# federicomegler/sq-learn

Hardware: AMD Instinct MI355X
Metric: q-means fit samples/sec (Lloyd samples*iterations/s, delta-means + tomography noise) (higher is better)
Workload: dtype fp32; 1 GPU; model=q-means k=1024 delta=0.5 (10000000 x 256 synthetic), global_batch=10000000, seq_len=256, parallelism=dp1

## Files before the change

sq_learn_amd/csrc/estep_f32.hip:

```cpp
#include "common.h"
#include "band.h"
#include "f16_tile.h"
#include "sq_api.h"

namespace sq {

constexpr int kMaxCand = 16;

#ifndef SQ_SPLIT_ACC_ALL
#define SQ_SPLIT_ACC_ALL 1
#endif
template <int KSD, int TOP = 2>
__global__ void __launch_bounds__(256, 1) estep_f32_kernel(
    const float* __restrict__ X, const _Float16* __restrict__ C, const float* __restrict__ xn,
    int* __restrict__ labels, float* __restrict__ mind, long long* __restrict__ ovf_rows,
    int* __restrict__ ovf_count, double* __restrict__ part, long long n, int k_pad, float alpha,
    float inv_alpha2, float delta_s, RngKey key, long long row_offset, int ovf_cap,
    const long long* __restrict__ rlist, const int* __restrict__ rcount,
    const float* __restrict__ cmax2_p, long long* __restrict__ mrows, int* __restrict__ mcand,
    int* __restrict__ multi_count, unsigned char* __restrict__ xflag, long long mcap) {
  const float Cm = cmax2_p ? sqrtf(*cmax2_p) * (1.0f + 0x1p-16f) : 0.0f;
  constexpr bool SPLIT_ACC = SQ_SPLIT_ACC_ALL || TOP == 3;
  constexpr float kEps3 =
      SPLIT_ACC ? (3.0f * 0x1p-22f + (KSD * 16 + 18.0f) * 0x1p-24f + 2.0f * KSD * 16 * 0x1p-34f) *
// ... 1310 lines not shown
      const unsigned long long pm = __ballot(cin && rank == r) & gmask;
      if (wide && pm) plane = __ffsll((long long)pm) - 1;
      dmin_w = mine ? dme : __builtin_inff();
#pragma unroll
      for (int o = 1; o < LPR; o <<= 1) dmin_w = fminf(dmin_w, __shfl_xor(dmin_w, o, 64));
    }
    const int pick = __shfl(cur.myj, plane, 64);
    const float hpick = __shfl(hi, plane, 64);
    const float dpick = __shfl(dme, plane, 64);
    float lo_o = (mine && lane != plane) ? lo : __builtin_inff();
#pragma unroll
    for (int o = 1; o < LPR; o <<= 1) lo_o = fminf(lo_o, __shfl_xor(lo_o, o, 64));
    fix(nxt);
    ldrow(Cm + (size_t)nxt.j0 * DX, c0n);
    ldrow(Cm + (size_t)nxt.j1 * DX, c1n);
    __builtin_amdgcn_sched_barrier(0);
    labels[g] = pick;
    if constexpr (UB) ub[g] = sqrtf(hpick) * (1.0f + 0x1p-20f);
    if (wide && sub == 0 && corr) corr[g] = dmin_w - dpick;
    xflag[e] = done_any ? 0 : 1;
    if (rec) {
      const float dpl = __shfl(dme, plane, 64), spl = __shfl(slack, plane, 64);
      const float gc = mine ? dme - dpl : 0.0f;
      float ge = mine ? slack + spl + fabsf(gc) * 0x1p-23f : 0.0f;
#pragma unroll
      for (int o = 1; o < LPR; o <<= 1) ge = fmaxf(ge, __shfl_xor(ge, o, 64));
      const int w = sub & 7;
      const float gw = __shfl(gc, gbase + min(max(w - 2, 0), LPR - 1), 64);
      const float v = w == 0 ? dpl : (w == 1 ? ge : gw);
      const unsigned i0 = (unsigned)__shfl(cur.myj, gbase, 64) & 0x3FFFu;
      const unsigned i1 = (unsigned)__shfl(cur.myj, gbase + 1, 64) & 0x3FFFu;
      const unsigned i2 = (unsigned)__shfl(cur.myj, gbase + 2, 64) & 0x3FFFu;
      const unsigned i3 = (unsigned)__shfl(cur.myj, gbase + 3, 64) & 0x3FFFu;
      const unsigned cm1 = (unsigned)min(max(c_r, 1), kGapCand) - 1u;
      const unsigned id0 = i0 | ((unsigned)(plane - gbase) & 3u) << 14 |
                           (c_r > 1 ? i1 : i0) << 16 | cm1 << 30;
      const unsigned id1 = (c_r > 2 ? i2 : i0) | (c_r > 3 ? i3 : i0) << 16;
      float* rw = reinterpret_cast<float*>(rec + g) + w;
      if (w < 6) *rw = v;
      else *reinterpret_cast<unsigned*>(rw) = w == 6 ? id0 : id1;
      if (sub == 0) rec_it[g] = (done && c_r <= kGapCand) ? it_now + 2 : 1;
    }
    __builtin_amdgcn_sched_barrier(0);
    g2 = g3;
    g3 = g4;
  };
  for (long long st = 0; st < nsteps; st += 2) {
    step(st, rA, xA, c0A, c1A, rB, xB, c0B, c1B);
    if (st + 1 >= nsteps) break;
    step(st + 1, rB, xB, c0B, c1B, rA, xA, c0A, c1A);
  }
}

typedef _Float16 gs_h2 __attribute__((ext_vector_type(2)));
__device__ __forceinline__ float gs_dot(const uint4 a, const uint4 b, float acc) {
  acc = __builtin_amdgcn_fdot2(__builtin_bit_cast(gs_h2, a.x), __builtin_bit_cast(gs_h2, b.x), acc,
                               false);
  acc = __builtin_amdgcn_fdot2(__builtin_bit_cast(gs_h2, a.y), __builtin_bit_cast(gs_h2, b.y), acc,
                               false);
  acc = __builtin_amdgcn_fdot2(__builtin_bit_cast(gs_h2, a.z), __builtin_bit_cast(gs_h2, b.z), acc,
                               false);
  acc = __builtin_amdgcn_fdot2(__builtin_bit_cast(gs_h2, a.w), __builtin_bit_cast(gs_h2, b.w), acc,
                               false);
  return acc;
}
__device__ __forceinline__ float gs_dot(const uint2 a, const uint2 b, float acc) {
  acc = __builtin_amdgcn_fdot2(__builtin_bit_cast(gs_h2, a.x), __builtin_bit_cast(gs_h2, b.x), acc,
                               false);
  acc = __builtin_amdgcn_fdot2(__builtin_bit_cast(gs_h2, a.y), __builtin_bit_cast(gs_h2, b.y), acc,
                               false);
  return acc;
}
__device__ __forceinline__ uint4 gs_zero(uint4) { return make_uint4(0u, 0u, 0u, 0u); }
template <int CTRL>
__device__ __forceinline__ float gs_dpp_add(float v) {
  return v + __int_as_float(__builtin_amdgcn_update_dpp(0, __float_as_int(v), CTRL, 0xF, 0xF,
                                                         false));
}
__device__ __forceinline__ uint2 gs_zero(uint2) { return make_uint2(0u, 0u); }

template <int DX>
__global__ void __launch_bounds__(256) gap_screen_kernel(
    const _Float16* __restrict__ Xh, const float* __restrict__ xn,
    const long long* __restrict__ mrows_b, const int* __restrict__ count_b,
    const _Float16* __restrict__ dsh, long long dsh_stride, const float* __restrict__ dq,
    long long dq_stride, float inv_alpha, float delta, int* __restrict__ labels,
    GapRec* __restrict__ rec, int* __restrict__ mflag, int it_now, int ring, int rebase_age,
    long long* __restrict__ mrows, int* __restrict__ multi_count, long long cap,
    int* __restrict__ n_done, long long* __restrict__ mrows_mv, int* __restrict__ count_mv) {
  constexpr int LPR = 32;
  using VT = typename std::conditional<DX % 256 == 0, uint4, uint2>::type;
  constexpr int HV = (int)sizeof(VT) / 2;
  constexpr int V = DX / (LPR * HV);
  static_assert(DX % 128 == 0 && V >= 1, "gap screen: d_pad multiple of 128");
  const int lane = threadIdx.x & 63;
  const int sub = lane & (LPR - 1);
  const bool hi = lane >= LPR;
  const long long cnt = min((long long)*count_b, cap);
  const long long gw = (long long)blockIdx.x * (blockDim.x >> 6) + (threadIdx.x >> 6);
  const long long nw = (long long)gridDim.x * (blockDim.x >> 6);
  const long long nblk = (cnt + 63) / 64;
  const float sub_err = sqrtf((float)DX) * 0x1p-25f * inv_alpha;
  constexpr float gam = (float)(DX + 16) * 0x1p-24f;
  uint32_t done_cnt = 0;
  constexpr int kGapStage = 256;
  __shared__ long long stage_fw[4][kGapStage], stage_mv[4][kGapStage];
  int n_fw = 0, n_mv = 0;
  auto flush = [&](const long long* buf, int& cnt, long long* __restrict__ dst, int* counter) {
    if (cnt == 0) return;
    int b = 0;
    if (lane == 0) b = atomicAdd(counter, cnt);
    b = __shfl(b, 0, 64);
    __builtin_amdgcn_wave_barrier();
    for (int i = lane; i < cnt; i += 64)
      if ((long long)b + i < cap) dst[(long long)b + i] = buf[i];
    cnt = 0;
  };
  auto stage = [&](bool pred, long long row, long long* buf, int& cnt, long long* __restrict__ dst,
                   int* counter) {
    const unsigned long long pm = __ballot(pred);
    if (pm == 0) return;
    if (cnt + 64 > kGapStage) flush(buf, cnt, dst, counter);
    if (pred) buf[cnt + __popcll(pm & ((1ull << lane) - 1ull))] = row;
    cnt += __popcll(pm);
  };
  auto rl = [](int v, int l) -> int { return __builtin_amdgcn_readlane(v, l); };
  auto rlf = [](float v, int l) -> float {
    return __int_as_float(__builtin_amdgcn_readlane(__float_as_int(v), l));
  };
  for (long long blk = gw; blk < nblk; blk += nw) {
    const long long e = blk * 64 + lane;
    const bool live = e < cnt;
    const long long g = mrows_b[live ? e : cnt - 1];
    const int base_it = mflag[g] - 2;
    const int rslot = base_it % ring, age = it_now - base_it;
    const float4* rp = reinterpret_cast<const float4*>(rec + g);
    const float4 r0 = rp[0], r1 = rp[1];
    const float xq = xn[g];
    const unsigned id0 = __float_as_uint(r1.z), id1 = __float_as_uint(r1.w);
    const int c_r = (int)(id0 >> 30) + 1, slot = (int)((id0 >> 14) & 3u);
    int jc[kGapCand];
    jc[0] = (int)(id0 & 0x3FFFu);
    jc[1] = (int)((id0 >> 16) & 0x3FFFu);
    jc[2] = (int)(id1 & 0x3FFFu);
    jc[3] = (int)((id1 >> 16) & 0x3FFFu);
    const float* dqs = dq + (size_t)rslot * dq_stride;
    float4 d0[kGapCand];
    float inv[kGapCand];
#pragma unroll
    for (int c = 0; c < kGapCand; ++c) {
      d0[c] = reinterpret_cast<const float4*>(dqs)[2 * jc[c]];
      inv[c] = dqs[8 * jc[c] + 4];
    }
    float y[kGapCand] = {0.0f, 0.0f, 0.0f, 0.0f};
    constexpr int NB = 4;
    VT xv[NB][V], sv[NB][kGapCand][V];
    int pcm[NB];
    auto issue = [&](int p, int b) {
      const int ra = 2 * p, rb = 2 * p + 1;
      const long long ga = ((long long)rl((int)(g >> 32), ra) << 32) | (unsigned)rl((int)g, ra);
      const long long gb = ((long long)rl((int)(g >> 32), rb) << 32) | (unsigned)rl((int)g, rb);
      const long long gm = hi ? gb : ga;
      const VT* xr = reinterpret_cast<const VT*>(Xh + (size_t)gm * DX);
#pragma unroll
      for (int q = 0; q < V; ++q) xv[b][q] = xr[q * LPR + sub];
      const int sa = rl(rslot, ra), sb = rl(rslot, rb);
      const _Float16* ds = dsh + (size_t)(hi ? sb : sa) * dsh_stride;
      pcm[b] = max(rl(c_r, ra), rl(c_r, rb));
#pragma unroll
      for (int c = 0; c < kGapCand; ++c) {
        if (c < 2 || c < pcm[b]) {
          const int j = hi ? rl(jc[c], rb) : rl(jc[c], ra);
          const VT* sr = reinterpret_cast<const VT*>(ds + (size_t)j * DX);
#pragma unroll
          for (int q = 0; q < V; ++q) sv[b][c][q] = sr[q * LPR + sub];
        } else {
#pragma unroll
          for (int q = 0; q < V; ++q) sv[b][c][q] = gs_zero(VT{});
        }
      }
    };
    auto consume = [&](int p, int b) {
#pragma unroll
      for (int c = 0; c < kGapCand; ++c) {
        if (c < 2 || c < pcm[b]) {
          float acc = 0.0f;
#pragma unroll
          for (int q = 0; q < V; ++q) acc = gs_dot(xv[b][q], sv[b][c][q], acc);
          acc = gs_dpp_add<0xB1>(acc);
          acc = gs_dpp_add<0x4E>(acc);
          acc = gs_dpp_add<0x141>(acc);
          acc = gs_dpp_add<0x140>(acc);
          const float a = rlf(acc, 0) + rlf(acc, 16), bb = rlf(acc, 32) + rlf(acc, 48);
          y[c] = lane == 2 * p ? a : (lane == 2 * p + 1 ? bb : y[c]);
        }
      }
    };
#pragma unroll
    for (int b = 0; b < NB - 1; ++b) issue(b, b);
#pragma unroll 1
    for (int p = 0; p < 32; p += NB) {
#pragma unroll
      for (int b = 0; b < NB; ++b) {
        if (p + b + NB - 1 < 32) issue(p + b + NB - 1, (b + NB - 1) % NB);
        consume(p + b, b);
      }
    }
    const float nx = sqrtf(xq) * (1.0f + 0x1p-16f);
    const float ex = 0x1p-11f * nx + sub_err, nxh = nx + ex;
    float yr[kGapCand], E[kGapCand], qv[kGapCand];
#pragma unroll
    for (int c = 0; c < kGapCand; ++c) {
      yr[c] = y[c] * inv[c];
      E[c] = ex * d0[c].z + nxh * (d0[c].w + gam * (d0[c].z + d0[c].w)) + d0[c].y;
      qv[c] = d0[c].x;
    }
    float ya = 0.0f, Ea = 0.0f, qa = 0.0f;
#pragma unroll
    for (int c = 0; c < kGapCand; ++c)
      if (c == slot) {
        ya = yr[c];
        Ea = E[c];
        qa = qv[c];
      }
    const float gold[kGapCand] = {r0.z, r0.w, r1.x, r1.y};
    float gn[kGapCand], gmax = 0.0f, Emax = 0.0f, ymax = fabsf(ya), qmax = fabsf(qa);
#pragma unroll
    for (int c = 0; c < kGapCand; ++c) {
      const bool in = c < c_r;
      gn[c] = in ? (c == slot ? 0.0f : gold[c] + 2.0f * (ya - yr[c]) + (qv[c] - qa))
                 : __builtin_inff();
      if (in) {
        gmax = fmaxf(gmax, fabsf(gold[c]));
        Emax = fmaxf(Emax, E[c]);
        ymax = fmaxf(ymax, fabsf(yr[c]));
        qmax = fmaxf(qmax, fabsf(qv[c]));
      }
    }
    const float da = r0.x - 2.0f * ya + qa;
    float err = r0.y + 2.0f * (Ea + Emax) +
                0x1p-22f * (fmaxf(gmax, fabsf(r0.x)) + 4.0f * ymax + 2.0f * qmax);
    err *= 1.0f + 0x1p-20f;
    int m = 0;
    float gm = gn[0];
#pragma unroll
    for (int c = 1; c < kGapCand; ++c)
      if (gn[c] < gm) {
        gm = gn[c];
        m = c;
      }
    bool done = live && c_r >= 2 && slot < c_r && err < 0.25f * delta + 1.0f;
    float gmx = 0.0f;
#pragma unroll
    for (int c = 0; c < kGapCand; ++c)
      if (c < c_r && c != m) {
        done = done && (gn[c] - gm > delta + 2.0f * err);
        gmx = fmaxf(gmx, gn[c]);
      }
    if (done && (m != slot || age >= rebase_age)) {
      const float da_n = da + gm;
      float err_n =
          (m == slot ? err : 2.0f * err) + 0x1p-22f * (gmx + fabsf(da_n) + fabsf(gm));
      err_n *= 1.0f + 0x1p-20f;
      float gr[kGapCand];
#pragma unroll
      for (int c = 0; c < kGapCand; ++c) gr[c] = c < c_r ? gn[c] - gm : 0.0f;
      float4* wp = reinterpret_cast<float4*>(rec + g);
      wp[0] = make_float4(da_n, err_n, gr[0], gr[1]);
      wp[1] = make_float4(gr[2], gr[3],
                          __uint_as_float((id0 & ~(3u << 14)) | (unsigned)m << 14),
                          __uint_as_float(id1));
      if (m != slot) labels[g] = jc[0] * (m == 0) + jc[1] * (m == 1) + jc[2] * (m == 2) +
                                 jc[3] * (m == 3);
      mflag[g] = it_now + 2;
    }
    const bool fwd = live && !done;
    stage(fwd, g, stage_fw[threadIdx.x >> 6], n_fw, mrows, multi_count);
    if (mrows_mv)
      stage(fwd || (done && m != slot), g, stage_mv[threadIdx.x >> 6], n_mv, mrows_mv, count_mv);
    done_cnt += __popcll(__ballot(done));
  }
  flush(stage_fw[threadIdx.x >> 6], n_fw, mrows, multi_count);
  if (mrows_mv) flush(stage_mv[threadIdx.x >> 6], n_mv, mrows_mv, count_mv);
  if (n_done && lane == 0 && done_cnt) atomicAdd(n_done, (int)done_cnt);
}

__global__ void __launch_bounds__(256) shift_operand_kernel(
    const float* __restrict__ Cprev, const float* __restrict__ Cnew, int ldc, int d, int d_pad,
    int k, double alpha, float* __restrict__ snap, _Float16* __restrict__ dsh,
    float* __restrict__ dq, int snew, unsigned valid) {
  const int lane = threadIdx.x & 63;
  const int j = blockIdx.x * 4 + (threadIdx.x >> 6);
  const int sl = blockIdx.y;
  if (j >= k || !((valid >> sl) & 1u)) return;
  const size_t rs = (size_t)sl * k + j;
  const float* cn = Cnew + (size_t)j * ldc;
  float* sn = snap + rs * d_pad;
  const bool fresh = sl == snew;
  const float* co = fresh ? Cprev + (size_t)j * ldc : sn;
  double amax = 0.0;
  for (int f = lane; f < d; f += 64) amax = fmax(amax, fabs((double)cn[f] - (double)co[f]));
#pragma unroll
  for (int o = 32; o > 0; o >>= 1) amax = fmax(amax, __shfl_xor(amax, o, 64));
  int ex2 = 0;
  if (amax > 0.0) frexp(amax, &ex2);
  const double beta = amax > 0.0 ? ldexp(1.0, 14 - ex2) : 1.0;
  double q = 0.0, nrm = 0.0, nd = 0.0, e2 = 0.0;
  for (int f = lane; f < d_pad; f += 64) {
    const float a32 = f < d ? co[f] : 0.0f;
    const double a = (double)a32, b = f < d ? (double)cn[f] : 0.0;
    const double sft = b - a;
    const _Float16 h = (_Float16)(float)(beta * sft);
    dsh[rs * d_pad + f] = h;
    if (fresh) sn[f] = a32;
    const double r = sft - (double)h / beta;
    q += sft * (b + a);
    nrm += b * b + a * a;
    nd += sft * sft;
    e2 += r * r;
  }
#pragma unroll
  for (int o = 32; o > 0; o >>= 1) {
    q += __shfl_xor(q, o, 64);
    nrm += __shfl_xor(nrm, o, 64);
    nd += __shfl_xor(nd, o, 64);
    e2 += __shfl_xor(e2, o, 64);
// ... 140 lines not shown
      hi_at(d_pad + 2) = lo;
    }
  }
}

__global__ void __launch_bounds__(256) centers_f16_operand_kernel(const float* __restrict__ Cm,
                                                                  _Float16* __restrict__ op,
                                                                  int k, int d, int d_pad,
                                                                  float alpha) {
  __shared__ double red[4];
  const int j = blockIdx.x;
  write_f16_operand_row(op, j, k, Cm + (size_t)(j < k ? j : 0) * d, d, d_pad, alpha, threadIdx.x,
                        red);
}

}

using namespace sq;

template <int KSD, int TOP = 2>
static int launch_estep_f32(const void* X, const void* C, const void* xn, void* labels, void* mind,
                            void* ovf_rows, void* ovf_count, void* part, int part_cap,
                            void* inertia, long long n, int k_pad, float alpha, float inv_a2,
                            float delta_s, RngKey key, long long row_offset, int ovf_cap,
                            hipStream_t st, const void* rlist = nullptr,
                            const void* rcount = nullptr, const void* cmax2 = nullptr,
                            void* mrows = nullptr, void* mcand = nullptr,
                            void* multi_count = nullptr, void* xflag = nullptr,
                            long long mcap = 0) {
  constexpr int NW = 4;
  const size_t lds = 2 * (size_t)f16op::tile_bytes(KSD);
  auto kern = estep_f32_kernel<KSD, TOP>;
  static bool attr = false;
  if (!attr) {
    hipFuncSetAttribute((const void*)kern, hipFuncAttributeMaxDynamicSharedMemorySize, 160 * 1024);
    attr = true;
  }
  static int resident = 0;
  if (resident == 0) resident = resident_blocks((const void*)kern, NW * 64, lds);
  const long long nblk = (n + NW * 32 - 1) / (NW * 32);
  unsigned grid = (unsigned)(nblk < resident && !rlist ? nblk : resident);
  if ((long long)grid * NW > part_cap) grid = (unsigned)(part_cap / NW);
  if (grid == 0) return (int)hipErrorInvalidValue;
  hipLaunchKernelGGL(kern, dim3(grid), dim3(NW * 64), lds, st, (const float*)X,
                     (const _Float16*)C, (const float*)xn, (int*)labels, (float*)mind,
                     (long long*)ovf_rows, (int*)ovf_count, (double*)part, n, k_pad, alpha, inv_a2,
                     delta_s, key, row_offset, ovf_cap, (const long long*)rlist,
                     (const int*)rcount, (const float*)cmax2, (long long*)mrows, (int*)mcand,
                     (int*)multi_count, (unsigned char*)xflag, mcap);
  if (!inertia) return (int)hipGetLastError();
  return sq_sum_partials(part, (int)grid * NW, inertia, st);
}

template <int KSD>
static int launch_estep_x64(const void* Xh, const void* X, const void* C, const void* Cm,
                            const void* xn, const void* cmax2, void* labels, void* mind,
                            void* dense_rows, void* dense_count, void* mrows, void* mcand,
                            void* multi_count, void* corr, long long n, int k_pad, float alpha,
                            float delta_s, double delta, RngKey key, long long row_offset,
                            int dense_cap, hipStream_t st, const void* rlist, const void* rcount,
                            void* ub, void* lb, void* mflag, void* xflag, int list_rs,
                            const MultiRec& mrec, bool defer_rows = false) {
  int qbits = 1;
  while ((1 << qbits) < 2 * (k_pad / kTileN)) ++qbits;
  auto go = [&](auto RS_) {
    constexpr int RS = decltype(RS_)::value;
    constexpr int NW = kX64Waves;
    const size_t lds =
        (size_t)X64Ring<KSD>::BYTES + (size_t)NW * RS * 32 * (kMaxCand + 1) * 4 +
        (size_t)NW * 64 * 4;
    auto kern = estep_x64_kernel<KSD, RS>;
    static bool attr = false;
    if (!attr) {
      hipFuncSetAttribute((const void*)kern, hipFuncAttributeMaxDynamicSharedMemorySize,
                          160 * 1024);
      attr = true;
    }
    static int resident = 0;
    if (resident == 0) resident = resident_blocks((const void*)kern, NW * 64, lds);
    const long long nblk = (n + NW * 32 * RS - 1) / (NW * 32 * RS);
    const unsigned grid = (unsigned)(nblk < resident && !rlist ? nblk : resident);
    hipLaunchKernelGGL(kern, dim3(grid), dim3(NW * 64), lds, st, (const _Float16*)Xh,
                       (const float*)X, (const _Float16*)C, (const float*)Cm, (const float*)xn,
                       (const float*)cmax2, (int*)labels, (float*)mind, (long long*)dense_rows,
                       (int*)dense_count, (long long*)mrows, (int*)mcand, (int*)multi_count, n,
                       k_pad, alpha, delta_s, key, row_offset, dense_cap, qbits,
                       (const long long*)rlist, (const int*)rcount, (float*)ub, (float*)lb,
                       (int*)mflag);
  };
  static const bool list_rs1 = [] {
    const char* e = getenv("SQ_X64_LIST_RS1");
    return !(e && e[0] == '0');
  }();
  if (rlist && (list_rs == 1 || (list_rs == 0 && list_rs1)))
    go(std::integral_constant<int, 1>{});
  else
    go(std::integral_constant<int, X64RowSets<KSD>::value>{});
  int rc = (int)hipGetLastError();
  if (rc) return rc;
  const long long rblocks = (n / 16 + 63) / 64;
  const unsigned rgrid = (unsigned)(rblocks < 4096 ? (rblocks > 0 ? rblocks : 1) : 4096);
  if (xflag && mrec.rec && ub) {
    if constexpr (KSD * 16 % 128 == 0) {
      static long long gres = 0;
      if (gres == 0) {
        int dev = 0, cus = 0, per_cu = 0;
        hipGetDevice(&dev);
        hipDeviceGetAttribute(&cus, hipDeviceAttributeMultiprocessorCount, dev);
        hipOccupancyMaxActiveBlocksPerMultiprocessor(
            &per_cu, (const void*)gap_screen_kernel<KSD * 16>, 256, 0);
        gres = (long long)(cus > 0 ? cus : 256) * (per_cu > 0 ? per_cu : 2);
      }
      const unsigned bgrid = (unsigned)min(max(rblocks, 1LL), gres);
      hipLaunchKernelGGL(gap_screen_kernel<KSD * 16>, dim3(bgrid), dim3(256), 0, st,
                         (const _Float16*)Xh, (const float*)xn, mrec.mrows_b, mrec.count_b,
                         mrec.dsh, mrec.dsh_stride, mrec.dq,
                         mrec.dsh_stride / (KSD * 16) * 8, 1.0f / alpha, (float)delta,
                         (int*)labels, mrec.rec, mrec.mflag, mrec.it_now, mrec.ring,
                         max(1, mrec.ring / 2), (long long*)mrows, (int*)multi_count, n,
                         mrec.n_done, mrec.mrows_mv, mrec.count_mv);
    }
  }
  if (xflag) {
    static int sgrid = 0, sil = 0;
    if (sgrid == 0) {
      const char* ei = getenv("SQ_SCREEN_IL");
      sil = ei ? atoi(ei) : 0;
      const char* e = getenv("SQ_SCREEN_GRID");
      sgrid = e ? atoi(e) : 1024;
      if (sgrid <= 0) sgrid = 4096;
    }
    const unsigned fgrid2 = (unsigned)(rblocks < sgrid ? (rblocks > 0 ? rblocks : 1) : sgrid);
    auto fk = ub ? recheck_fast_kernel<KSD * 16, SQ_SCREEN_LPR, true>
                 : recheck_fast_kernel<KSD * 16, SQ_SCREEN_LPR, false>;
    hipLaunchKernelGGL(fk, dim3(fgrid2), dim3(256), 0, st, (const float*)X, (const float*)Cm,
                       (const long long*)mrows, (const int*)mcand, (const int*)multi_count,
                       (int*)labels, (float*)mind, n, delta, (float*)ub, (unsigned char*)xflag,
                       sil, mrec.rec, mrec.mflag, mrec.it_now, key, row_offset,
                       (float*)corr);
  }
  if (!defer_rows)
    hipLaunchKernelGGL(recheck_rows_kernel<KSD * 16>, dim3(rgrid), dim3(256), 0, st,
                       (const float*)X, (const float*)Cm, (const long long*)mrows,
                       (const int*)mcand, (const int*)multi_count, (int*)labels, (float*)mind, n,
                       delta, key, row_offset, (float*)corr, (float*)ub,
                       (const unsigned char*)xflag);
  return (int)hipGetLastError();
}

extern "C" {

int sq_estep_f32(const void* X, const void* C, const void* xn, void* labels, void* mind,
                 void* ovf_rows, void* ovf_count, void* part, int part_cap, void* inertia,
                 long long n, int d_pad, int k_pad, double alpha, double delta, unsigned k0,
                 unsigned k1, unsigned s0, unsigned s1, long long row_offset, int ovf_cap,
                 void* stream) {
  if (n <= 0) return 0;
  if (k_pad % kTileN != 0 || k_pad <= 0 || k_pad > 32768 || part_cap < 4)
    return (int)hipErrorInvalidValue;
  const double a2 = alpha * alpha;
  int aexp = 0;
  if (!(alpha > 0.0) || frexp(alpha, &aexp) != 0.5) return (int)hipErrorInvalidValue;
  RngKey key{k0, k1, s0, s1};
  hipStream_t st = (hipStream_t)stream;
  const float fa = (float)alpha, ia2 = (float)(1.0 / a2), ds = (float)(delta * a2);
  int rc;
  switch (d_pad) {
#define CASE(KSD)                                                                                \
  case KSD * 16:                                                                                 \
    rc = launch_estep_f32<KSD>(X, C, xn, labels, mind, ovf_rows, ovf_count, part, part_cap,      \
                               inertia, n, k_pad, fa, ia2, ds, key, row_offset, ovf_cap, st);    \
    break;
    CASE(1) CASE(2) CASE(4) CASE(8) CASE(16)
// ... 47 lines not shown
    rc = launch_estep_x64<KSD>(Xh, X, C, Cm, xn, cmax2, labels, mind, dense_rows, cnt + 1,       \
                               mrows, mcand, cnt + 2, corr, n, k_pad, fa, ds, delta, key,        \
                               row_offset, cap, st, rlist, rcount, ub, lb, mflag, xflag,         \
                               list_rs, mrec, true);                                             \
    if (rc) return rc;                                                                           \
    rc = launch_estep_f32<KSD>(X, C, xn, labels, mind, ovf_rows, cnt, part, part_cap, nullptr,   \
                               n, k_pad, fa, ia2, ds, key, row_offset, cap, st, dense_rows,       \
                               cnt + 1, cmax2, mrows, mcand, cnt + 2, xflag, n);                 \
    if (rc) return rc;                                                                           \
    if (ovf2.rows) {                                                                             \
                            \
                                                     \
      rc = launch_estep_f32<KSD, 3>(X, C, xn, labels, mind, ovf2.rows, ovf2.count, part,         \
                                    part_cap, nullptr, n, k_pad, fa, ia2, ds, key, row_offset,   \
                                    cap, st, ovf_rows, cnt, cmax2, mrows, mcand, cnt + 2, xflag, \
                                    n);                                                          \
      if (rc) return rc;                                                                         \
    }                                                                                            \
    if (corr)                                                                                    \
      hipLaunchKernelGGL(dense_corr_kernel, dim3(1024), dim3(256), 0, st, (const float*)X,       \
                         (const float*)Cm, (const long long*)dense_rows, (const int*)(cnt + 1),   \
                         (const int*)labels, (const float*)mind, (float*)corr, n, d_pad);        \
                        \
    hipLaunchKernelGGL(recheck_rows_kernel<KSD * 16>, dim3(rgrid), dim3(256), 0, st,            \
                       (const float*)X, (const float*)Cm, (const long long*)mrows,               \
                       (const int*)mcand, (const int*)(cnt + 2), (int*)labels, (float*)mind, n,  \
                       delta, key, row_offset, (float*)corr, (float*)ub,                         \
                       (const unsigned char*)xflag);                                             \
    rc = sq_rows_f64(X, d_pad, Cm, d_pad, d_pad, k, ovf2.rows ? ovf2.rows : ovf_rows,            \
                     ovf2.rows ? ovf2.count : cnt, 0, n, labels, mind, corr,                     \
                     ub, delta, k0, k1, s0, s1, row_offset, (int)fgrid, stream);                 \
    break;
    CASE(1) CASE(2) CASE(4) CASE(8) CASE(16)
#undef CASE
#define CASE(KSD)                                                                                \
  case KSD * 16:                                                                                 \
    rc = launch_estep_x64<KSD>(Xh, X, C, Cm, xn, cmax2, labels, mind, dense_rows, cnt + 1,       \
                               mrows, mcand, cnt + 2, corr, n, k_pad, fa, ds, delta, key,        \
                               row_offset, cap, st, rlist, rcount, ub, lb, mflag, xflag,         \
                               list_rs, mrec);                                                   \
    if (rc) return rc;                                                                           \
    rc = sq_rows_f64(X, d_pad, Cm, d_pad, d_pad, k, dense_rows, cnt + 1, 0, n, labels, mind,      \
                     corr, ub, delta, k0, k1, s0, s1, row_offset, (int)fgrid, stream);           \
    break;
    CASE(24) CASE(32) CASE(40) CASE(48) CASE(56) CASE(64)
#undef CASE
    default:
      return (int)hipErrorInvalidValue;
  }
  if (rc) return rc;
  return (int)hipGetLastError();
}

#if SQ_X64_STAMP
int sq_x64_stamps(void* host, int n_waves) {
  const int m = n_waves < kStampWaves ? n_waves : kStampWaves;
  return (int)hipMemcpyFromSymbol(host, HIP_SYMBOL(g_x64_stamps),
                                  (size_t)m * kStampN * sizeof(unsigned long long), 0,
                                  hipMemcpyDeviceToHost);
}
int sq_x64_stamps_clear() {
  static unsigned long long zeros[kStampWaves * kStampN];
  return (int)hipMemcpyToSymbol(HIP_SYMBOL(g_x64_stamps), zeros, sizeof(zeros), 0,
                                hipMemcpyHostToDevice);
}
#endif

int sq_fill_mind(const void* X, int ldx, const void* Cm, int d, const void* labels, void* mind,
                 long long n, void* stream) {
  if (n <= 0) return 0;
  const unsigned grid = (unsigned)((n + 3) / 4 < 8192 ? (n + 3) / 4 : 8192);
  hipLaunchKernelGGL(fill_mind_kernel, dim3(grid), dim3(256), 0, (hipStream_t)stream,
                     (const float*)X, ldx, (const float*)Cm, d, (const int*)labels, (float*)mind, n);
  return (int)hipGetLastError();
}

int sq_sum_f32(const void* v, long long n, void* part, int extra, void* out, void* stream) {
  hipStream_t st = (hipStream_t)stream;
  const int blocks = 512;
  if (extra < 0 || ((uintptr_t)v & 15u) != 0) return (int)hipErrorInvalidValue;
  hipLaunchKernelGGL(sum_f32_blocks_kernel, dim3(blocks), dim3(256), 0, st, (const float*)v, n,
                     (double*)part);
  return sq_sum_partials(part, blocks + extra, out, st);
}

int sq_centers_f16_operand(const void* Cm, void* op, int k, int d, int d_pad, int k_pad,
                           double alpha, void* stream) {
  if (k_pad % kTileN != 0 || d_pad % 16 != 0 || d > d_pad) return (int)hipErrorInvalidValue;
  hipLaunchKernelGGL(centers_f16_operand_kernel, dim3((unsigned)k_pad), dim3(256), 0,
                     (hipStream_t)stream, (const float*)Cm, (_Float16*)op, k, d, d_pad,
                     (float)alpha);
  return (int)hipGetLastError();
}

}
```

sq_learn_amd/csrc/sq_api.h:

```cpp
#pragma once

#ifndef SQ_API
#define SQ_API
#endif

extern "C" {

SQ_API int sq_trunc_normal_add(void* x, int dtype, long long n, double b, unsigned k0, unsigned k1,
                               unsigned s0, unsigned s1, unsigned long long offset, void* stream);
SQ_API int sq_philox_normal(void* out, int dtype, long long n, double mean, double stdv,
                            unsigned k0, unsigned k1, unsigned s0, unsigned s1,
                            unsigned long long offset, void* stream);
SQ_API int sq_philox_uniform(void* out, long long n, unsigned k0, unsigned k1, unsigned s0,
                             unsigned s1, unsigned long long offset, void* stream);
SQ_API int sq_ae_batch(const void* a, const void* eps, void* out, long long n, int Q, unsigned k0,
                       unsigned k1, unsigned s0, unsigned s1, unsigned long long offset,
                       void* stream);
SQ_API int sq_pe_batch(const void* omega, const void* m, void* out, long long n, unsigned k0,
                       unsigned k1, unsigned s0, unsigned s1, unsigned long long offset,
                       void* stream);

SQ_API int sq_tomography(const void* V, int r, int d, const void* sched, int T, int mode,
                         const void* first, void* err, void* out, int norm_inf, unsigned k0,
                         unsigned k1, unsigned s0, unsigned s1, long long row_offset, void* stream,
// ... 189 lines not shown
SQ_API int sq_kmpp_screen(void* closest, void* nearest, const void* mask_prev, const void* Dprev,
                          const void* best_prev, int c_prev, const void* cc, int ldcc, int t,
                          long long n, long long R, int G, void* mask_out, void* surv, void* exact,
                          void* scount, void* ecount, int prune, void* stream);
SQ_API int sq_kmpp_bound(const void* Xq, int dq, const void* srow, const void* erow,
                         const void* xq2, const void* closest, const void* candq,
                         const void* cinfo, int t, int d, long long n, long long R, int G,
                         const void* surv, const void* scount, void* exact, void* ecount,
                         void* stream);
SQ_API int sq_kmpp_dots(const void* Xq, int dq, long long n, const void* candq, void* out,
                        void* stream);
SQ_API int sq_kmpp_exact(const void* X, long long ldx, int d, long long n, int t, const void* cand,
                         const void* closest, const void* w, double scale, const void* exact,
                         const void* ecount, void* mask_out, void* Dout, void* delta_part,
                         long long R, int G, void* stream);
SQ_API int sq_kmpp_pick(const void* block_tot, int G, long long R, long long n, const void* vals,
                        int t, const void* closest, const void* mask, const void* D,
                        const void* best, const void* w, double scale, void* pos, const void* X,
                        long long ldx, int d, void* cands, void* cand_ids, long long row_offset,
                        long long n_global, void* stream);
SQ_API int sq_kmpp_finish(const void* delta_part, int G, int t, void* block_tot, void* P,
                          const void* draws_next, void* vals, const void* cands,
                          const void* cand_ids, int d, void* centers, void* ids, int c,
                          void* best_out, void* stream);
SQ_API int sq_kmpp_batch(int op, const long long* ia, void* stream);

SQ_API int sq_bounds_filter(const void* labels, void* ub, void* lb, const void* shift,
                            const void* smax, long long n, double delta, void* rlist, void* rcount,
                            const void* mflag, void* mrows, void* multi_count, const void* cc,
                            const void* fidx, int nf, int k, void* stream, void* corr,
                            void* rec_count, int rec_on, int it_now, int it_lo, void* mrows_b,
                            void* count_b);
SQ_API int sq_fast_centroids(void* shift, const void* shift_sq, const void* C, int k, int d, int nf,
                             void* idx, void* smax_rest, void* cc, void* stream);
SQ_API int sq_shift_operand(const void* Cprev, const void* Cnew, int ldc, int d, int d_pad, int k,
                            double alpha, void* snap, void* dsh, void* dq, int ring, int snew,
                            unsigned valid, void* stream);
SQ_API int sq_estep_f32(const void* X, const void* C, const void* xn, void* labels, void* mind,
                        void* ovf_rows, void* ovf_count, void* part, int part_cap, void* inertia,
                        long long n, int d_pad, int k_pad, double alpha, double delta, unsigned k0,
                        unsigned k1, unsigned s0, unsigned s1, long long row_offset, int ovf_cap,
                        void* stream);
SQ_API int sq_estep_x64(const void* Xh, const void* X, const void* C, const void* Cm,
                        const void* xn, const void* cmax2, void* labels, void* mind,
                        void* dense_rows, void* ovf_rows, void* mrows, void* mcand, void* corr,
                        void* rlist, void* rcount, void* ub, void* lb, void* mflag, void* xflag,
                        void* counts, void* part, int part_cap, long long n, int d, int d_pad,
                        int k, int k_pad, double alpha, double delta, unsigned k0, unsigned k1,
                        unsigned s0, unsigned s1, long long row_offset, int list_rs, void* stream,
                        void* rec, void* rec_mflag, int it_now, int it_lo, int ring,
                        const void* dsh, const void* dq, long long dsh_stride, void* mrows_b,
                        void* count_b, void* n_done, void* mrows_mv, void* count_mv,
                        void* ovf2_rows, void* ovf2_count);
SQ_API int sq_x64_stamps(void* host, int n_waves);
SQ_API int sq_x64_stamps_clear();
SQ_API int sq_fill_mind(const void* X, int ldx, const void* Cm, int d, const void* labels,
                        void* mind, long long n, void* stream);
SQ_API int sq_sum_f32(const void* v, long long n, void* part, int extra, void* out, void* stream);
SQ_API int sq_centers_f16_operand(const void* Cm, void* op, int k, int d, int d_pad, int k_pad,
                                  double alpha, void* stream);

SQ_API int sq_rows_f64(const void* X, long long ldx, const void* C, long long ldc, int d, int k,
                       const void* rows, const void* count, long long n_direct, long long cap,
                       void* labels, void* mind, void* corr, void* ub, double delta, unsigned k0,
                       unsigned k1, unsigned s0, unsigned s1, long long row_offset, int grid,
                       void* stream);

SQ_API int sq_mu_sums(const void* X, int xdtype, long long ldx, const void* qs, int nq,
                      void* rowmax, void* colsum, void* part, int part_wgs, void* rowacc,
                      long long n, int d, const void* mean, float qstep, void* stream);
SQ_API int sq_col_moments(const void* X, int xdtype, long long ldx, long long n, int d, void* part,
                          int part_wgs, void* stream);
SQ_API int sq_row_norms(const void* X, int xdtype, void* out, long long n, int d, void* stream);

SQ_API int sq_knn_topk(const void* D, void* outd, void* outi, long long m, int nref, long long ldD,
                       int kk, long long col_offset, void* stream);

}
```

sq_learn_amd/ops/kmeans.py:

```python

import math
import os
from typing import NamedTuple

import numpy as np

import torch

from ..runtime.rng import RngKey, philox4x32, MASK32
from . import _native as nat
from .random import amplitude_estimation_batch

FAST_D = (16, 32, 64, 128, 256)
X64_D = FAST_D + (384, 512, 640, 768, 896, 1024)
X64_MAX_K = 16384
BIG = 3.0e38


def pad_features(d):
    for f in X64_D:
        if d <= f:
            return f
    return ((d + 15) // 16) * 16

# ... 311 lines not shown
    assert shift.numel() >= k and shift.is_contiguous()
    if shift_sq is not None:
        assert shift_sq.dtype == torch.float64 and shift_sq.is_contiguous() and shift_sq.numel() >= k
    nat.native().fast_centroids(shift.data_ptr(),
                                0 if shift_sq is None else shift_sq.data_ptr(), C.data_ptr(),
                                k, d, int(nf), idx.data_ptr(), smax_rest.data_ptr(),
                                cc.data_ptr(), nat.stream_handle(C.device))


class MultiRecords(NamedTuple):
    rec: int
    mflag: int
    it_now: int
    it_lo: int
    ring: int
    dsh: int
    dq: int
    dsh_stride: int
    rows_b: int
    count_b: int
    n_done: int
    rows_moved: int
    count_moved: int


def multi_records(rec=None, mflag=None, it_now=0, it_lo=0, dsh=None, dq=None, rows_b=None,
                  count_b=None, n_done=None, rows_moved=None, count_moved=None):
    if rec is None:
        return None
    assert rec.dtype == torch.float32 and rec.shape[-1] == 8 and mflag.dtype == torch.int32
    assert dsh.dtype == torch.float16 and dq.dtype == torch.float32 and rows_b.dtype == torch.int64
    assert dsh.dim() == 3 and dq.shape[:2] == dsh.shape[:2] and dq.shape[2] == 8
    if rows_moved is not None:
        assert rows_moved.dtype == torch.int64 and rows_moved.numel() >= rows_b.numel()
        assert count_moved.dtype == torch.int32
    return MultiRecords(rec.data_ptr(), mflag.data_ptr(), int(it_now), int(it_lo),
                        int(dsh.shape[0]), dsh.data_ptr(), dq.data_ptr(), int(dsh.stride(0)),
                        rows_b.data_ptr(), count_b.data_ptr(),
                        0 if n_done is None else n_done.data_ptr(),
                        0 if rows_moved is None else rows_moved.data_ptr(),
                        0 if rows_moved is None else count_moved.data_ptr())


def shift_operand_native(C_prev, C_new, alpha, snap, dsh, dq, snew, valid):
    k, d = C_new.shape[0], C_new.shape[1]
    ring, _, d_pad = dsh.shape
    assert C_prev.dtype == torch.float32 and C_new.dtype == torch.float32
    assert C_prev.stride() == C_new.stride() and C_new.stride(1) == 1
    assert tuple(snap.shape) == (ring, k, d_pad) and tuple(dq.shape) == (ring, k, 8)
    nat.native().shift_operand(C_prev.data_ptr(), C_new.data_ptr(), int(C_new.stride(0)), int(d),
                               int(d_pad), int(k), float(alpha), snap.data_ptr(), dsh.data_ptr(),
                               dq.data_ptr(), int(ring), int(snew), int(valid),
                               nat.stream_handle(C_new.device))


def ensure_multi_buffers(buf: EStepBuffers, n, device, bounds=False):
    if buf.dense_rows is None or buf.dense_rows.numel() < n:
        buf.dense_rows = torch.empty(max(n, 1), dtype=torch.int64, device=device)
    if buf.multi_rows is None or buf.multi_rows.numel() < n:
        buf.multi_rows = torch.empty(max(n, 1), dtype=torch.int64, device=device)
        buf.multi_cand = torch.empty((max(n, 1), 17), dtype=torch.int32, device=device)
    if bounds and (buf.mflag is None or buf.mflag.numel() < n):
        buf.mflag = torch.zeros(max(n, 1), dtype=torch.int32, device=device)


def centroid_delta_native(X, labels, prev, sums, counts, qsum, k, ws: ReduceWorkspace, perm2,
                          qexp, lists=None):
    n, d = X.shape
    assert X.dtype == torch.float32 and X.is_contiguous() and d % 4 == 0 and d <= 1024
    assert labels.dtype == torch.int32 and prev.dtype == torch.int32 and perm2.numel() >= 4 * n
    assert sums.dtype == torch.float64 and sums.numel() >= k * d and qsum.numel() >= k
    if lists is not None:
        lp = []
        for ent in list(lists) + [None] * (3 - len(lists)):
            if ent is None:
                lp += [0, 0]
            else:
                rows, cnt = ent
                assert rows.dtype == torch.int64 and cnt.dtype == torch.int32
                lp += [rows.data_ptr(), cnt.data_ptr()]
        nat.native().centroid_delta_lists(X.data_ptr(), labels.data_ptr(), prev.data_ptr(),
                                          sums.data_ptr(), counts.data_ptr(),
                                          qsum.data_ptr(), n, d, k, ws.xexp, int(qexp),
                                          ws.hist.data_ptr(), ws.cursor.data_ptr(),
                                          perm2.data_ptr(), *lp, nat.stream_handle(X.device))
        return
    nat.native().centroid_delta(X.data_ptr(), labels.data_ptr(), prev.data_ptr(),
                                sums.data_ptr(), counts.data_ptr(), qsum.data_ptr(), n, d, k,
                                ws.xexp, int(qexp), ws.hist.data_ptr(), ws.cursor.data_ptr(),
                                perm2.data_ptr(), nat.stream_handle(X.device))


def cluster_inertia_native(sums, counts, qsum, C, k, d, ws: ReduceWorkspace, qexp, part):
    assert C.dtype == torch.float32 and C.is_contiguous() and tuple(C.shape) == (k, d)
    nat.native().cluster_inertia(sums.data_ptr(), counts.data_ptr(), qsum.data_ptr(),
                                 C.data_ptr(), k, d, ws.xexp, int(qexp), part.data_ptr(),
                                 nat.stream_handle(C.device))


def mstep_stats_native(sums, counts, qsum, C, k, d, ws: ReduceWorkspace, qexp, corr, n, part,
                       inertia, packed):
    assert C.dtype == torch.float32 and C.is_contiguous() and tuple(C.shape) == (k, d)
    assert part.numel() >= 512 + k and part.dtype == torch.float64
    assert corr.dtype == torch.float32 and corr.data_ptr() % 16 == 0
    nat.native().mstep_stats(sums.data_ptr(), counts.data_ptr(), qsum.data_ptr(),
                             C.data_ptr(), k, d, ws.xexp, int(qexp), corr.data_ptr(), int(n),
# ... 814 lines not shown
```

Measured before the change: 16.20 billion samples*iter/s.

## Restructure gap-screen kernel issue pipeline with bpermute addressing and occupancy hint

Rewrites the gap screen kernel's load-issue path. Row and candidate offsets are now broadcast with ds_bpermute instead of readlane pairs, and candidate widening uses wave ballots. Dot products are separated from the DPP reductions, and the dq/xn metadata loads are deferred until just before the last pipeline group to ease register pressure. It also adds a launch-bounds occupancy hint for small DX, plus a standalone sq_gap_screen entry point with an optional debug output, which adds a per-row null check in the kernel. The risk is that the changed row-to-lane mapping, 32-bit offsets and heavier vector-register use interact in ways that are hard to predict.

```diff
diff --git a/sq_learn_amd/csrc/estep_f32.hip b/sq_learn_amd/csrc/estep_f32.hip
--- a/sq_learn_amd/csrc/estep_f32.hip
+++ b/sq_learn_amd/csrc/estep_f32.hip
@@ -1386,6 +1386,12 @@
   }
 }
 
+#ifndef SQ_GAP_ISSUE
+#define SQ_GAP_ISSUE 1
+#endif
+#ifndef SQ_GAP_REDUCE
+#define SQ_GAP_REDUCE 1
+#endif
 typedef _Float16 gs_h2 __attribute__((ext_vector_type(2)));
 __device__ __forceinline__ float gs_dot(const uint4 a, const uint4 b, float acc) {
   acc = __builtin_amdgcn_fdot2(__builtin_bit_cast(gs_h2, a.x), __builtin_bit_cast(gs_h2, b.x), acc,
@@ -1412,16 +1418,16 @@
                                                          false));
 }
 __device__ __forceinline__ uint2 gs_zero(uint2) { return make_uint2(0u, 0u); }
-
 template <int DX>
-__global__ void __launch_bounds__(256) gap_screen_kernel(
+__global__ void __launch_bounds__(256, DX <= 256 ? 3 : 1) gap_screen_kernel(
     const _Float16* __restrict__ Xh, const float* __restrict__ xn,
     const long long* __restrict__ mrows_b, const int* __restrict__ count_b,
     const _Float16* __restrict__ dsh, long long dsh_stride, const float* __restrict__ dq,
     long long dq_stride, float inv_alpha, float delta, int* __restrict__ labels,
     GapRec* __restrict__ rec, int* __restrict__ mflag, int it_now, int ring, int rebase_age,
     long long* __restrict__ mrows, int* __restrict__ multi_count, long long cap,
-    int* __restrict__ n_done, long long* __restrict__ mrows_mv, int* __restrict__ count_mv) {
+    int* __restrict__ n_done, long long* __restrict__ mrows_mv, int* __restrict__ count_mv,
+    float* __restrict__ ydbg) {
   constexpr int LPR = 32;
   using VT = typename std::conditional<DX % 256 == 0, uint4, uint2>::type;
   constexpr int HV = (int)sizeof(VT) / 2;
@@ -1429,7 +1435,6 @@
   static_assert(DX % 128 == 0 && V >= 1, "gap screen: d_pad multiple of 128");
   const int lane = threadIdx.x & 63;
   const int sub = lane & (LPR - 1);
-  const bool hi = lane >= LPR;
   const long long cnt = min((long long)*count_b, cap);
   const long long gw = (long long)blockIdx.x * (blockDim.x >> 6) + (threadIdx.x >> 6);
   const long long nw = (long long)gridDim.x * (blockDim.x >> 6);
@@ -1458,10 +1463,12 @@
     if (pred) buf[cnt + __popcll(pm & ((1ull << lane) - 1ull))] = row;
     cnt += __popcll(pm);
   };
+#if !SQ_GAP_ISSUE || SQ_GAP_REDUCE
   auto rl = [](int v, int l) -> int { return __builtin_amdgcn_readlane(v, l); };
   auto rlf = [](float v, int l) -> float {
     return __int_as_float(__builtin_amdgcn_readlane(__float_as_int(v), l));
   };
+#endif
   for (long long blk = gw; blk < nblk; blk += nw) {
     const long long e = blk * 64 + lane;
     const bool live = e < cnt;
@@ -1470,7 +1477,6 @@
     const int rslot = base_it % ring, age = it_now - base_it;
     const float4* rp = reinterpret_cast<const float4*>(rec + g);
     const float4 r0 = rp[0], r1 = rp[1];
-    const float xq = xn[g];
     const unsigned id0 = __float_as_uint(r1.z), id1 = __float_as_uint(r1.w);
     const int c_r = (int)(id0 >> 30) + 1, slot = (int)((id0 >> 14) & 3u);
     int jc[kGapCand];
@@ -1478,20 +1484,49 @@
     jc[1] = (int)((id0 >> 16) & 0x3FFFu);
     jc[2] = (int)(id1 & 0x3FFFu);
     jc[3] = (int)((id1 >> 16) & 0x3FFFu);
-    const float* dqs = dq + (size_t)rslot * dq_stride;
-    float4 d0[kGapCand];
-    float inv[kGapCand];
-#pragma unroll
-    for (int c = 0; c < kGapCand; ++c) {
-      d0[c] = reinterpret_cast<const float4*>(dqs)[2 * jc[c]];
-      inv[c] = dqs[8 * jc[c] + 4];
-    }
     float y[kGapCand] = {0.0f, 0.0f, 0.0f, 0.0f};
     constexpr int NB = 4;
     VT xv[NB][V], sv[NB][kGapCand][V];
+#if SQ_GAP_ISSUE
+    const int xlo = (int)(unsigned)g, xhi = (int)(unsigned)((unsigned long long)g >> 32);
+    int coff[kGapCand];
+#pragma unroll
+    for (int c = 0; c < kGapCand; ++c)
+      coff[c] = (int)(unsigned)(((size_t)rslot * dsh_stride + (size_t)jc[c] * DX) * 2);
+    const unsigned long long b2 = __ballot(c_r > 2), b3 = __ballot(c_r > 3);
+    const unsigned wide2 = (unsigned)(b2 | (b2 >> 32)), wide3 = (unsigned)(b3 | (b3 >> 32));
+    auto wide = [&](int c, int p, int) -> bool {
+      return c < 2 || (((c == 2 ? wide2 : wide3) >> p) & 1u) != 0;
+    };
+    auto issue = [&](int p, int b) __attribute__((always_inline)) {
+      const int src = ((lane & LPR) + p) << 2;
+      auto bc = [&](int v) -> unsigned { return (unsigned)__builtin_amdgcn_ds_bpermute(src, v); };
+      const char* xr = reinterpret_cast<const char*>(Xh) +
+                       ((((unsigned long long)bc(xhi) << 32) | bc(xlo)) * (DX * 2) +
+                        sub * sizeof(VT));
+#pragma unroll
+      for (int q = 0; q < V; ++q)
+        xv[b][q] = *reinterpret_cast<const VT*>(xr + q * LPR * (int)sizeof(VT));
+#pragma unroll
+      for (int c = 0; c < kGapCand; ++c) {
+        if (wide(c, p, b)) {
+          const unsigned o = bc(coff[c]) + (unsigned)(sub * (int)sizeof(VT));
+          const char* sr = reinterpret_cast<const char*>(dsh) + o;
+#pragma unroll
+          for (int q = 0; q < V; ++q)
+            sv[b][c][q] = *reinterpret_cast<const VT*>(sr + q * LPR * (int)sizeof(VT));
+        } else {
+#pragma unroll
+          for (int q = 0; q < V; ++q) sv[b][c][q] = gs_zero(VT{});
+        }
+      }
+    };
+#else
     int pcm[NB];
-    auto issue = [&](int p, int b) {
-      const int ra = 2 * p, rb = 2 * p + 1;
+    auto wide = [&](int c, int, int b) -> bool { return c < 2 || c < pcm[b]; };
+    auto issue = [&](int p, int b) __attribute__((always_inline)) {
+      const int ra = p, rb = 32 + p;
+      const bool hi = lane >= LPR;
       const long long ga = ((long long)rl((int)(g >> 32), ra) << 32) | (unsigned)rl((int)g, ra);
       const long long gb = ((long long)rl((int)(g >> 32), rb) << 32) | (unsigned)rl((int)g, rb);
       const long long gm = hi ? gb : ga;
@@ -1503,7 +1538,7 @@
       pcm[b] = max(rl(c_r, ra), rl(c_r, rb));
 #pragma unroll
       for (int c = 0; c < kGapCand; ++c) {
-        if (c < 2 || c < pcm[b]) {
+        if (wide(c, p, b)) {
           const int j = hi ? rl(jc[c], rb) : rl(jc[c], ra);
           const VT* sr = reinterpret_cast<const VT*>(ds + (size_t)j * DX);
 #pragma unroll
@@ -1514,32 +1549,62 @@
         }
       }
     };
-    auto consume = [&](int p, int b) {
+#endif
+    auto dots = [&](int b, float (&acc)[kGapCand]) __attribute__((always_inline)) {
 #pragma unroll
       for (int c = 0; c < kGapCand; ++c) {
-        if (c < 2 || c < pcm[b]) {
-          float acc = 0.0f;
-#pragma unroll
-          for (int q = 0; q < V; ++q) acc = gs_dot(xv[b][q], sv[b][c][q], acc);
-          acc = gs_dpp_add<0xB1>(acc);
-          acc = gs_dpp_add<0x4E>(acc);
-          acc = gs_dpp_add<0x141>(acc);
-          acc = gs_dpp_add<0x140>(acc);
-          const float a = rlf(acc, 0) + rlf(acc, 16), bb = rlf(acc, 32) + rlf(acc, 48);
-          y[c] = lane == 2 * p ? a : (lane == 2 * p + 1 ? bb : y[c]);
+        acc[c] = 0.0f;
+#pragma unroll
+        for (int q = 0; q < V; ++q) acc[c] = gs_dot(xv[b][q], sv[b][c][q], acc[c]);
+      }
+    };
+#pragma unroll
+    for (int b = 0; b < NB - 1; ++b) issue(b, b);
+    auto group = [&](const int p, auto TAIL_) __attribute__((always_inline)) {
+      constexpr bool TAIL = decltype(TAIL_)::value;
+#pragma unroll
+      for (int b = 0; b < NB; ++b) {
+        __builtin_amdgcn_sched_barrier(0);
+        if (!TAIL || b == 0) issue(p + b + NB - 1, (b + NB - 1) % NB);
+        float acc[kGapCand];
+        dots(b, acc);
+#pragma unroll
+        for (int c = 0; c < kGapCand; ++c) asm volatile("" : "+v"(acc[c]));
+#if SQ_GAP_REDUCE
+#pragma unroll
+        for (int c = 0; c < kGapCand; ++c) {
+          if (wide(c, p + b, b)) {
+            float a = acc[c];
+            a = gs_dpp_add<0xB1>(a);
+            a = gs_dpp_add<0x4E>(a);
+            a = gs_dpp_add<0x141>(a);
+            a = gs_dpp_add<0x140>(a);
+            const float lo = rlf(a, 0) + rlf(a, 16), up = rlf(a, 32) + rlf(a, 48);
+            y[c] = lane == p + b ? lo : (lane == 32 + p + b ? up : y[c]);
+          }
         }
+#else
+#pragma unroll
+        for (int c = 0; c < kGapCand; ++c) y[c] += acc[c];
+#endif
       }
     };
-#pragma unroll
-    for (int b = 0; b < NB - 1; ++b) issue(b, b);
 #pragma unroll 1
-    for (int p = 0; p < 32; p += NB) {
-#pragma unroll
-      for (int b = 0; b < NB; ++b) {
-        if (p + b + NB - 1 < 32) issue(p + b + NB - 1, (b + NB - 1) % NB);
-        consume(p + b, b);
-      }
-    }
+    for (int p = 0; p < 32 - NB; p += NB) group(p, std::false_type{});
+    unsigned il0 = id0, il1 = id1;
+    asm volatile("" : "+v"(il0), "+v"(il1));
+    const int jl[kGapCand] = {(int)(il0 & 0x3FFFu), (int)((il0 >> 16) & 0x3FFFu),
+                              (int)(il1 & 0x3FFFu), (int)((il1 >> 16) & 0x3FFFu)};
+    const float xq = xn[g];
+    const float* dqs = dq + (size_t)rslot * dq_stride;
+    float4 d0[kGapCand];
+    float inv[kGapCand];
+#pragma unroll
+    for (int c = 0; c < kGapCand; ++c) {
+      d0[c] = reinterpret_cast<const float4*>(dqs)[2 * jl[c]];
+      inv[c] = dqs[8 * jl[c] + 4];
+    }
+    group(32 - NB, std::true_type{});
     const float nx = sqrtf(xq) * (1.0f + 0x1p-16f);
     const float ex = 0x1p-11f * nx + sub_err, nxh = nx + ex;
     float yr[kGapCand], E[kGapCand], qv[kGapCand];
@@ -1548,6 +1613,11 @@
       yr[c] = y[c] * inv[c];
       E[c] = ex * d0[c].z + nxh * (d0[c].w + gam * (d0[c].z + d0[c].w)) + d0[c].y;
       qv[c] = d0[c].x;
+    }
+    if (ydbg && live) {
+#pragma unroll
+      for (int c = 0; c < kGapCand; ++c)
+        if (c < c_r) ydbg[e * kGapCand + c] = yr[c];
     }
     float ya = 0.0f, Ea = 0.0f, qa = 0.0f;
 #pragma unroll
@@ -1604,8 +1674,8 @@
       wp[1] = make_float4(gr[2], gr[3],
                           __uint_as_float((id0 & ~(3u << 14)) | (unsigned)m << 14),
                           __uint_as_float(id1));
-      if (m != slot) labels[g] = jc[0] * (m == 0) + jc[1] * (m == 1) + jc[2] * (m == 2) +
-                                 jc[3] * (m == 3);
+      if (m != slot) labels[g] = jl[0] * (m == 0) + jl[1] * (m == 1) + jl[2] * (m == 2) +
+                                 jl[3] * (m == 3);
       mflag[g] = it_now + 2;
     }
     const bool fwd = live && !done;
@@ -1852,6 +1922,34 @@
   return sq_sum_partials(part, (int)grid * NW, inertia, st);
 }
 
+template <int DX>
+static int launch_gap_screen(const void* Xh, const void* xn, const MultiRec& mrec, float inv_alpha,
+                             float delta, void* labels, void* mrows, void* multi_count,
+                             long long cap, long long rblocks, int grid_blocks, void* ydbg,
+                             hipStream_t st) {
+  if (mrec.dsh_stride <= 0 || mrec.dsh_stride % DX != 0 ||
+      (unsigned long long)mrec.ring * (unsigned long long)mrec.dsh_stride * 2ull >= (1ull << 32))
+    return (int)hipErrorInvalidValue;
+  static long long gres = 0;
+  if (gres == 0) {
+    int dev = 0, cus = 0, per_cu = 0;
+    hipGetDevice(&dev);
+    hipDeviceGetAttribute(&cus, hipDeviceAttributeMultiprocessorCount, dev);
+    hipOccupancyMaxActiveBlocksPerMultiprocessor(&per_cu, (const void*)gap_screen_kernel<DX>, 256,
+                                                 0);
+    gres = (long long)(cus > 0 ? cus : 256) * (per_cu > 0 ? per_cu : 2);
+  }
+  const unsigned bgrid =
+      grid_blocks > 0 ? (unsigned)grid_blocks : (unsigned)min(max(rblocks, 1LL), gres);
+  hipLaunchKernelGGL(gap_screen_kernel<DX>, dim3(bgrid), dim3(256), 0, st, (const _Float16*)Xh,
+                     (const float*)xn, mrec.mrows_b, mrec.count_b, mrec.dsh, mrec.dsh_stride,
+                     mrec.dq, mrec.dsh_stride / DX * 8, inv_alpha, delta, (int*)labels, mrec.rec,
+                     mrec.mflag, mrec.it_now, mrec.ring, max(1, mrec.ring / 2), (long long*)mrows,
+                     (int*)multi_count, cap, mrec.n_done, mrec.mrows_mv, mrec.count_mv,
+                     (float*)ydbg);
+  return (int)hipGetLastError();
+}
+
 template <int KSD>
 static int launch_estep_x64(const void* Xh, const void* X, const void* C, const void* Cm,
                             const void* xn, const void* cmax2, void* labels, void* mind,
@@ -1902,23 +2000,9 @@
   const unsigned rgrid = (unsigned)(rblocks < 4096 ? (rblocks > 0 ? rblocks : 1) : 4096);
   if (xflag && mrec.rec && ub) {
     if constexpr (KSD * 16 % 128 == 0) {
-      static long long gres = 0;
-      if (gres == 0) {
-        int dev = 0, cus = 0, per_cu = 0;
-        hipGetDevice(&dev);
-        hipDeviceGetAttribute(&cus, hipDeviceAttributeMultiprocessorCount, dev);
-        hipOccupancyMaxActiveBlocksPerMultiprocessor(
-            &per_cu, (const void*)gap_screen_kernel<KSD * 16>, 256, 0);
-        gres = (long long)(cus > 0 ? cus : 256) * (per_cu > 0 ? per_cu : 2);
-      }
-      const unsigned bgrid = (unsigned)min(max(rblocks, 1LL), gres);
-      hipLaunchKernelGGL(gap_screen_kernel<KSD * 16>, dim3(bgrid), dim3(256), 0, st,
-                         (const _Float16*)Xh, (const float*)xn, mrec.mrows_b, mrec.count_b,
-                         mrec.dsh, mrec.dsh_stride, mrec.dq,
-                         mrec.dsh_stride / (KSD * 16) * 8, 1.0f / alpha, (float)delta,
-                         (int*)labels, mrec.rec, mrec.mflag, mrec.it_now, mrec.ring,
-                         max(1, mrec.ring / 2), (long long*)mrows, (int*)multi_count, n,
-                         mrec.n_done, mrec.mrows_mv, mrec.count_mv);
+      rc = launch_gap_screen<KSD * 16>(Xh, xn, mrec, 1.0f / alpha, (float)delta, labels, mrows,
+                                       multi_count, n, rblocks, 0, nullptr, st);
+      if (rc) return rc;
     }
   }
   if (xflag) {
@@ -2072,6 +2156,35 @@
   return (int)hipGetLastError();
 }
 
+int sq_gap_screen(const void* Xh, const void* xn, const void* mrows_b, const void* count_b,
+                  const void* dsh, const void* dq, long long dsh_stride, int ring, double alpha,
+                  double delta, void* labels, void* rec, void* rec_mflag, int it_now, void* mrows,
+                  void* multi_count, void* n_done, void* mrows_mv, void* count_mv, long long n,
+                  int d_pad, int grid_blocks, void* ydbg, void* stream) {
+  if ((mrows_mv != nullptr) != (count_mv != nullptr)) return (int)hipErrorInvalidValue;
+  if (!Xh || !xn || !mrows_b || !count_b || !dsh || !dq || !labels || !rec || !rec_mflag ||
+      !mrows || !multi_count || it_now < 1 || ring < 2 || ring > 16 || grid_blocks < 0)
+    return (int)hipErrorInvalidValue;
+  int aexp = 0;
+  if (!(alpha > 0.0) || frexp(alpha, &aexp) != 0.5) return (int)hipErrorInvalidValue;
+  if (n <= 0) return 0;
+  const MultiRec mrec{(GapRec*)rec, (int*)rec_mflag, it_now, it_now, ring, (const _Float16*)dsh,
+                      (const float*)dq, dsh_stride, (long long*)mrows_b, (int*)count_b,
+                      (int*)n_done, (long long*)mrows_mv, (int*)count_mv};
+  const long long rblocks = (n / 16 + 63) / 64;
+  hipStream_t st = (hipStream_t)stream;
+  switch (d_pad) {
+#define CASE(DX)                                                                                 \
+  case DX:                                                                                       \
+    return launch_gap_screen<DX>(Xh, xn, mrec, (float)(1.0 / alpha), (float)delta, labels, mrows, \
+                                 multi_count, n, rblocks, grid_blocks, ydbg, st);
+    CASE(128) CASE(256) CASE(384) CASE(512) CASE(640) CASE(768) CASE(896) CASE(1024)
+#undef CASE
+    default:
+      return (int)hipErrorInvalidValue;
+  }
+}
+
 #if SQ_X64_STAMP
 int sq_x64_stamps(void* host, int n_waves) {
   const int m = n_waves < kStampWaves ? n_waves : kStampWaves;
diff --git a/sq_learn_amd/csrc/sq_api.h b/sq_learn_amd/csrc/sq_api.h
--- a/sq_learn_amd/csrc/sq_api.h
+++ b/sq_learn_amd/csrc/sq_api.h
@@ -265,6 +265,12 @@
                         const void* dsh, const void* dq, long long dsh_stride, void* mrows_b,
                         void* count_b, void* n_done, void* mrows_mv, void* count_mv,
                         void* ovf2_rows, void* ovf2_count);
+SQ_API int sq_gap_screen(const void* Xh, const void* xn, const void* mrows_b, const void* count_b,
+                         const void* dsh, const void* dq, long long dsh_stride, int ring,
+                         double alpha, double delta, void* labels, void* rec, void* rec_mflag,
+                         int it_now, void* mrows, void* multi_count, void* n_done, void* mrows_mv,
+                         void* count_mv, long long n, int d_pad, int grid_blocks, void* ydbg,
+                         void* stream);
 SQ_API int sq_x64_stamps(void* host, int n_waves);
 SQ_API int sq_x64_stamps_clear();
 SQ_API int sq_fill_mind(const void* X, int ldx, const void* Cm, int d, const void* labels,
diff --git a/sq_learn_amd/ops/kmeans.py b/sq_learn_amd/ops/kmeans.py
--- a/sq_learn_amd/ops/kmeans.py
+++ b/sq_learn_amd/ops/kmeans.py
@@ -387,6 +387,41 @@
                                int(d_pad), int(k), float(alpha), snap.data_ptr(), dsh.data_ptr(),
                                dq.data_ptr(), int(ring), int(snew), int(valid),
                                nat.stream_handle(C_new.device))
+
+
+_GAP_SCREEN = None
+
+
+def _gap_screen_entry():
+    global _GAP_SCREEN
+    if _GAP_SCREEN is None:
+        import ctypes
+        P, L, I, D = ctypes.c_void_p, ctypes.c_longlong, ctypes.c_int, ctypes.c_double
+        fn = ctypes.CDLL(nat.loaded_path()).sq_gap_screen
+        fn.restype = I
+        fn.argtypes = [P, P, P, P, P, P, L, I, D, D, P, P, P, I, P, P, P, P, P, L, I, I, P, P]
+        _GAP_SCREEN = fn
+    return _GAP_SCREEN
+
+
+def gap_screen_native(Xh, xn, labels, multi_rows, multi_count, records: MultiRecords, alpha,
+                      delta, grid_blocks=0, ydbg=None):
+    n, d_pad = Xh.shape
+    assert Xh.dtype == torch.float16 and Xh.is_contiguous() and xn.dtype == torch.float32
+    assert labels.dtype == torch.int32 and multi_rows.dtype == torch.int64
+    assert multi_rows.numel() >= n and multi_count.dtype == torch.int32
+    if ydbg is not None:
+        assert ydbg.dtype == torch.float32 and ydbg.is_contiguous() and ydbg.numel() >= 4 * n
+    r = records
+    p = lambda a: a or None
+    rc = _gap_screen_entry()(
+        Xh.data_ptr(), xn.data_ptr(), r.rows_b, r.count_b, r.dsh, r.dq, r.dsh_stride, r.ring,
+        float(alpha), float(delta), labels.data_ptr(), r.rec, r.mflag, r.it_now,
+        multi_rows.data_ptr(), multi_count.data_ptr(), p(r.n_done), p(r.rows_moved),
+        p(r.count_moved), int(n), int(d_pad), int(grid_blocks), p(nat.ptr(ydbg)),
+        p(nat.stream_handle(Xh.device)))
+    if rc != 0:
+        raise RuntimeError(f"sq_learn_amd native launch failed: sq_gap_screen ({rc})")
 
 
 def ensure_multi_buffers(buf: EStepBuffers, n, device, bounds=False):
```

Measured after the change: 16.70 billion samples*iter/s, median of 6. 3.1% higher.
